# Gadersd/stable-diffusion-burn

Measured on NVIDIA H100. Metric: images_per_sec_512x512_20steps, higher is better.
Workload: dtype fp16 tensor-core operands (3-term split-fp16 on the two high-res UNet levels), fp32 accumulate

## Files before the change

### stable_diffusion_burn_b200/csrc/api.cu

```cuda
#include "../../include/sdb200.h"

#include <dlfcn.h>

#include <cstdlib>
#include <cstring>
#include <mutex>

#include "attention.cuh"
#include "kernels.cuh"
#include "model.cuh"
#include "runtime.cuh"

using namespace sdb;

struct sdb_ctx {
  Ctx c;
};

static thread_local std::string g_err;

#define API_BEGIN(ctxp)                      \
  if (!(ctxp)) {                             \
    g_err = "null context";                  \
    return 1;                                \
// ... 323 lines not shown
                    int L, const float* d_uncond, int Lu, double guidance_scale, int n_steps, const float* d_noise, int H, int W,
                    float* d_latent_out, uint8_t* d_rgb_out, void* stream) {
  API_BEGIN(ctx)
  need_final(c);
  model_img2img_dev(c, d_image, d_mask, strength, d_context, n, L, d_uncond, Lu, guidance_scale, n_steps, d_noise, H, W,
                    d_latent_out, d_rgb_out, (cudaStream_t)stream);
  API_END
}

int sdb_forward_diffuser(sdb_ctx* ctx, const float* latent, int32_t timestep, const float* context, int n, int L,
                         const float* uncond, int Lu, double guidance_scale, int H, int W, float* pred, float* out_uncond,
                         float* out_cond) {
  API_BEGIN(ctx)
  need_final(c);
  SDB_CHECK(latent && context && uncond, "null argument");
  model_forward_diffuser_host(c, latent, timestep, context, n, L, uncond, Lu, guidance_scale, H, W, pred, out_uncond, out_cond);
  API_END
}

int sdb_forward_diffuser_dev(sdb_ctx* ctx, const float* d_latent, int32_t timestep, const float* d_context, int n, int L,
                             const float* d_uncond, int Lu, double guidance_scale, int H, int W, float* d_pred, void* stream) {
  API_BEGIN(ctx)
  need_final(c);
  model_forward_diffuser_dev(c, d_latent, timestep, d_context, n, L, d_uncond, Lu, guidance_scale, H, W, d_pred, nullptr, nullptr,
                             (cudaStream_t)stream);
  API_END
}

int sdb_encode_image(sdb_ctx* ctx, const float* img, int n, int H, int W, float* latent) {
  API_BEGIN(ctx)
  need_final(c);
  SDB_CHECK(img && latent, "null argument");
  model_encode_host(c, img, n, H, W, latent);
  API_END
}

int sdb_encode_image_dev(sdb_ctx* ctx, const float* d_img, int n, int H, int W, float* d_latent, void* stream) {
  API_BEGIN(ctx)
  need_final(c);
  model_encode_dev(c, d_img, n, H, W, d_latent, (cudaStream_t)stream);
  API_END
}

int sdb_clip_forward(sdb_ctx* ctx, const int32_t* tokens, int n, int L, float* out) {
  API_BEGIN(ctx)
  need_final(c);
  SDB_CHECK(tokens && out, "null argument");
  model_clip_forward_host(c, tokens, n, L, out);
  API_END
}

int sdb_clip_forward_dev(sdb_ctx* ctx, const int32_t* d_tokens, int n, int L, float* d_out, void* stream) {
  API_BEGIN(ctx)
  need_final(c);
  model_clip_forward_dev(c, d_tokens, n, L, d_out, (cudaStream_t)stream);
  API_END
}

int sdb_set_option(sdb_ctx* ctx, const char* key, int value) {
  API_BEGIN(ctx)
  const std::string k = key ? key : "";
  if (k == "precision")
    c.opt_precision = value;
  else if (k == "graphs")
    c.opt_graphs = value;
  else if (k == "splitk")
    c.opt_splitk = value;
  else if (k == "raw16")
    c.opt_raw16 = value;
  else if (k == "splitk_min_iters")
    c.opt_splitk_min_iters = value;
  else if (k == "splitk_chunk")
    c.opt_splitk_chunk = value < 1 ? 1 : value;
  else if (k == "attn_split")
    c.opt_attn_split = value;
  else if (k == "attn_regsplit")
    g_attn_regsplit = value;
  else if (k == "emb_hoist")
    c.opt_emb_hoist = value;
  else if (k == "prefetch_w")
    c.opt_prefetch_w = value;
  else if (k == "mlp_passes")
    c.opt_mlp_passes = value;
  else if (k == "gn_epilogue")
    c.opt_gn_epilogue = value;
  else if (k == "skip_merge")
    c.opt_skip_merge = value;
  else if (k == "gn_apply_ctas")
    g_gn_apply_ctas = value < 1 ? 1 : value;
  else if (k == "gn_min_pix")
    g_gn_min_pix = value < 1 ? 1 : value;
  else
    throw Error("unknown option: " + k);
  model_invalidate_graphs(c);
  API_END
}

int sdb_profile_enable(sdb_ctx* ctx, int on) {
  API_BEGIN(ctx)
  profile_collect(c);
  c.profiling = on != 0;
  API_END
}
int sdb_profile_reset(sdb_ctx* ctx) {
  API_BEGIN(ctx)
  profile_collect(c);
  c.launches = 0;
  for (int i = 0; i < KC_COUNT; ++i) c.cls_ms[i] = c.cls_flops[i] = c.cls_bytes[i] = c.cls_issued[i] = 0, c.cls_launches[i] = 0;
  API_END
}
int sdb_profile_class_count(sdb_ctx*) { return KC_COUNT; }
int sdb_profile_get(sdb_ctx* ctx, int cls, const char** name, int64_t* launches, double* ms, double* flops, double* bytes) {
  API_BEGIN(ctx)
  SDB_CHECK(cls >= 0 && cls < KC_COUNT, "class index");
  profile_collect(c);
  if (name) *name = kernel_class_name(cls);
  if (launches) *launches = c.cls_launches[cls];
  if (ms) *ms = c.cls_ms[cls];
  if (flops) *flops = c.cls_flops[cls];
  if (bytes) *bytes = c.cls_bytes[cls];
  API_END
}
int sdb_profile_get_issued(sdb_ctx* ctx, int cls, double* issued_flops) {
  API_BEGIN(ctx)
  SDB_CHECK(cls >= 0 && cls < KC_COUNT && issued_flops, "class index");
  *issued_flops = c.cls_issued[cls];
  API_END
}
int64_t sdb_launch_count(sdb_ctx* ctx) { return ctx ? ctx->c.launches : -1; }

int sdb_test_linear(sdb_ctx* ctx, const float* a, const float* w, const float* bias, int M, int K, int N, int passes,
                    float* out) {
  API_BEGIN(ctx)
  c.work.reset();
  float* d_a = c.work.get<float>((size_t)M * K);
  float* d_w = c.work.get<float>((size_t)K * N);
  float* d_b = bias ? c.work.get<float>(N) : nullptr;
  float* d_c = c.work.get<float>((size_t)M * N);
  SDB_CUDA(cudaMemcpyAsync(d_a, a, sizeof(float) * M * K, cudaMemcpyHostToDevice, c.stream));
  SDB_CUDA(cudaMemcpyAsync(d_w, w, sizeof(float) * K * N, cudaMemcpyHostToDevice, c.stream));
  if (bias) SDB_CUDA(cudaMemcpyAsync(d_b, bias, sizeof(float) * N, cudaMemcpyHostToDevice, c.stream));
  ActOp A;
  A.p.hi = c.work.get<__half>((size_t)M * K);
  A.p.lo = c.work.get<__half>((size_t)M * K);
  A.W = M, A.C = K;
  WeightOp Wp;
  Wp.p.hi = c.work.get<__half>((size_t)N * K);
  Wp.p.lo = c.work.get<__half>((size_t)N * K);
  Wp.N = N, Wp.K = K;
  convert_f16_launch(d_a, (long long)M * K, A.p, c.stream);
  pack_linear_launch(d_w, K, N, Wp.p, 0, c.stream);
  Epilogue ep;
  ep.out_f32 = d_c;
  ep.bias = d_b;
  run_gemm(c, G_LINEAR, A, nullptr, Wp, passes, ep);
  SDB_CUDA(cudaMemcpyAsync(out, d_c, sizeof(float) * M * N, cudaMemcpyDeviceToHost, c.stream));
  SDB_CUDA(cudaStreamSynchronize(c.stream));
  API_END
}

int sdb_test_gemm_ex(sdb_ctx* ctx, const float* a, const float* w, const float* bias, const float* residual, int M, int K, int N,
                     int passes, int flags, const float* xa, const float* xw, int XK, float* out) {
  API_BEGIN(ctx)
  c.work.reset();
  const bool geglu = flags & 1, from_f16 = flags & 4;
  SDB_CHECK(!geglu || (N % 128 == 0 && !residual && !xa), "GEGLU test: N (= 2 * hidden) must be a multiple of 128, no residual / extra K");
// ... 321 lines not shown
```

### stable_diffusion_burn_b200/csrc/gemm_tc.cu

```cuda
#include "gemm_tc.cuh"

#include <cstring>

namespace sdb {

static constexpr int BM = 128;
static constexpr int BK = 64;
static constexpr int A_TILE_BYTES = BM * BK * 2;

template <int BN, int PASSES>
struct StageLayout {
  static constexpr int B_TILE_BYTES = BN * BK * 2;
  static constexpr int A_TILES = PASSES >= 2 ? 2 : 1;
  static constexpr int B_TILES = PASSES >= 3 ? 2 : 1;
  static constexpr int BYTES = A_TILES * A_TILE_BYTES + B_TILES * B_TILE_BYTES;
};
template <int BN>
struct AccLayout {
  static constexpr int PITCH = (BN + 4) * 4;
  static constexpr int BYTES = BM * PITCH;
  static constexpr int GN_BYTES = 32 * 1024;
};
static constexpr int EW = 8;

// ... 559 lines not shown
      if constexpr (kGN) {
        asm volatile("bar.sync 1, %0;" ::"n"(EW * 32) : "memory");
        gn_write_partials(p, gn_cs, BN, threadIdx.x - 128, EW * 32, gnt, col0, p.up2 ? (int)blockIdx.z * p.gn_phase_slots : 0);
      }
    }
    if (dbg && threadIdx.x == 128) dbg[6] = clock64();
  }
  __syncthreads();
  if (dbg && threadIdx.x == 0) dbg[7] = clock64();
}

static constexpr int SMEM_OPTIN_MAX = 227 * 1024;
template <int BN, int PASSES>
constexpr int pick_stages() {
  constexpr int per = StageLayout<BN, PASSES>::BYTES;
  constexpr int n = (SMEM_OPTIN_MAX - 1024) / (per + 2 * 8);
  return n > 8 ? 8 : n;
}

template <int BN, int PASSES, int STAGES, int EPI>
static void launch_epi(const GemmMaps& maps, const GemmParams& p, cudaStream_t stream) {
  constexpr int smem = region_bytes<BN, PASSES, STAGES>() + 2 * STAGES * 8 + 1024;
  static_assert(smem <= SMEM_OPTIN_MAX, "shared memory per block");
  static_assert(4 * BN * 8 <= AccLayout<BN>::GN_BYTES && 2 * (EW * 32) * 4 * 16 <= AccLayout<BN>::GN_BYTES,
                "GroupNorm column sums must fit in the scratch after the accumulator image");
  static DeviceOnce once;
  if (once.first())
    SDB_CUDA(cudaFuncSetAttribute(gemm_tc_kernel<BN, PASSES, STAGES, EPI>, cudaFuncAttributeMaxDynamicSharedMemorySize, smem));
  dim3 grid(p.tiles_n * p.tiles_h * p.tiles_w, (p.N + BN - 1) / BN, p.up2 ? 4 : p.split_k);
  launch_k(gemm_tc_kernel<BN, PASSES, STAGES, EPI>, grid, dim3(128 + 32 * EW), (size_t)smem, stream, maps, p);
}
template <int BN, int PASSES, int STAGES>
static void launch_inst(const GemmMaps& maps, const GemmParams& p, cudaStream_t stream) {
  SDB_CHECK((p.gn_part != nullptr) + (p.ln_out != nullptr) + (p.ln_in != nullptr) <= 1, "one statistics role per launch");
  if constexpr (BN == 128) {
    if (p.geglu) {
      SDB_CHECK(!p.gn_part && !p.ln_out && p.split_k == 1, "GEGLU epilogue: no statistics output, no split-K");
      return p.ln_in ? launch_epi<BN, PASSES, STAGES, EPI_GEGLU_LNC>(maps, p, stream)
                     : launch_epi<BN, PASSES, STAGES, EPI_GEGLU>(maps, p, stream);
    }
  }
  SDB_CHECK(!p.geglu, "the GEGLU epilogue is built for 128-wide tiles");
  if constexpr (BN >= 128) {
    if (p.gn_part) return launch_epi<BN, PASSES, STAGES, EPI_GN>(maps, p, stream);
  }
  if constexpr (BN == 160) {
    if (p.ln_out) return launch_epi<BN, PASSES, STAGES, EPI_LNS>(maps, p, stream);
  }
  if constexpr (BN == 128 || BN == 160) {
    if (p.ln_in) return launch_epi<BN, PASSES, STAGES, EPI_LNC>(maps, p, stream);
  }
  SDB_CHECK(!p.gn_part && !p.ln_out && !p.ln_in, "this statistics epilogue is not built for this tile width");
  launch_epi<BN, PASSES, STAGES, EPI_PLAIN>(maps, p, stream);
}
bool gemm_tc_supports(int BN, int epi) {
  return epi == EPI_PLAIN || (epi == EPI_GN && BN >= 128) || (epi == EPI_LNS && BN == 160) || (epi == EPI_LNC && (BN == 128 || BN == 160));
}

template <int BN, int PASSES>
static void launch_bn(const GemmMaps& maps, const GemmParams& p, cudaStream_t stream) {
  launch_inst<BN, PASSES, pick_stages<BN, PASSES>()>(maps, p, stream);
}

void gemm_tc_launch(const GemmMaps& maps, const GemmParams& p, int BN, int passes, cudaStream_t stream) {
  SDB_CHECK(p.TN * p.TH * p.TW == BM, "M tile must cover 128 rows");
  SDB_CHECK(p.N % 32 == 0, "N must be a multiple of 32");
#define SDB_DISPATCH(bn)                                             \
  case bn:                                                           \
    if (passes == 1) launch_bn<bn, 1>(maps, p, stream);              \
    else if (passes == 2) launch_bn<bn, 2>(maps, p, stream);         \
    else launch_bn<bn, 3>(maps, p, stream);                          \
    break;
  switch (BN) {
    SDB_DISPATCH(64)
    SDB_DISPATCH(128)
    SDB_DISPATCH(160)
    SDB_DISPATCH(256)
    default:
      throw Error("unsupported BN");
  }
#undef SDB_DISPATCH
}

}
```

### stable_diffusion_burn_b200/csrc/gemm_tc.cuh

```cuda
#pragma once
#include "common.cuh"

namespace sdb {

struct GemmMaps {
  CUtensorMap a[4][2];
  CUtensorMap bx[2];
  CUtensorMap b[2];
};

struct GemmParams {
  int nimg, H, W;
  int TN, TH, TW;
  int tiles_n, tiles_h, tiles_w;
  int N;
  int kc;
  int kc0;
  int num_taps;
  int xkc, xkc0;
  int8_t tap_dh[9], tap_dw[9], tap_ph[9];
  int split_k;
  int up2, gn_phase_slots;
  float* out_f32;
  __half* out_f16;
  __half* out_f16_lo;
  const float* bias;
  const float* rowbias;
  const float* residual;
  int ldc;
  int ldc16;
  int geglu;
  long long* dbg;
  int prefetch_w;
  int pdl_late;
  int act;
  float* gn_part;
  int gn_cap, gn_bucket, gn_slot0;
  int gn_rpi, gn_nimg;
  float* ln_out;
  int ln_slots;
  const float* ln_in;
  int ln_in_slots, ln_C;
  float ln_eps;
  const float* ln_u;
  const __half* res_hi;
  const __half* res_lo;
  float* ws;
  unsigned int* tickets;
  int OH, OW, os, oa, ob;
};

struct GemmLaunch {
  int BN, passes, stages;
};

void gemm_tc_launch(const GemmMaps& maps, const GemmParams& p, int BN, int passes, cudaStream_t stream);
bool gemm_tc_supports(int BN, int epi);
int gemm_tc_smem_bytes(int BN, int passes, int stages);

}
```

### stable_diffusion_burn_b200/csrc/runtime.cu

```cuda
#include "runtime.cuh"

#include <algorithm>

#include <cudaTypedefs.h>

#include <cmath>
#include <cstdlib>
#include <cstring>

namespace sdb {

int g_pdl_late = 1;
bool g_pdl_enabled = true;
int g_num_sms = 132;

void Arena::init(size_t bytes) {
  SDB_CUDA(cudaMalloc(&base, bytes));
  cap = bytes;
  off = 0;
}
void Arena::destroy() {
  if (base) cudaFree(base);
  base = nullptr;
  cap = off = 0;
// ... 242 lines not shown
      p.num_taps = 9;
      for (int t = 0; t < 9; ++t) p.tap_dh[t] = t / 3 - 1, p.tap_dw[t] = t % 3 - 1, p.tap_ph[t] = 0;
      break;
    case G_CONV3_S2:
      SDB_CHECK(a0.P == 4, "stride-2 conv needs a 4-phase operand");
      p.num_taps = 9;
      for (int t = 0; t < 9; ++t) {
        const int kh = t / 3, kw = t % 3;
        p.tap_dh[t] = kh == 0 ? -1 : 0;
        p.tap_dw[t] = kw == 0 ? -1 : 0;
        p.tap_ph[t] = (kh != 1 ? 2 : 0) + (kw != 1 ? 1 : 0);
      }
      break;
    case G_CONV3_S2_PAD01:
      SDB_CHECK(a0.P == 4, "stride-2 conv needs a 4-phase operand");
      p.num_taps = 9;
      for (int t = 0; t < 9; ++t) {
        const int kh = t / 3, kw = t % 3;
        p.tap_dh[t] = kh == 2 ? 1 : 0;
        p.tap_dw[t] = kw == 2 ? 1 : 0;
        p.tap_ph[t] = (kh == 1 ? 2 : 0) + (kw == 1 ? 1 : 0);
      }
      break;
    case G_CONV3_UP2:
      p.num_taps = 4;
      phases_out = 4;
      break;
    default:
      throw Error("bad gemm kind");
  }
  SDB_CHECK(w.K == p.num_taps * Ctot, "weight K does not match the operand");
  if (xk) {
    const int xC = xk->x0.C + (xk->has_x1 ? xk->x1.C : 0);
    SDB_CHECK(kind == G_CONV3 || kind == G_LINEAR, "extra-K operands need an unshifted output grid");
    SDB_CHECK(xk->x0.n == a0.n && xk->x0.H == a0.H && xk->x0.W == a0.W && xk->x0.P == 1 && xk->x0.C % 64 == 0, "extra-K geometry");
    SDB_CHECK(!xk->has_x1 || (xk->x1.n == a0.n && xk->x1.H == a0.H && xk->x1.W == a0.W && xk->x1.C % 64 == 0), "extra-K geometry");
    SDB_CHECK(xk->w.N == w.N && xk->w.K == xC, "extra-K weights");
    SDB_CHECK(passes < 2 || (xk->x0.p.lo && (!xk->has_x1 || xk->x1.p.lo)), "multi-pass GEMM needs the lo half of the extra operands");
    SDB_CHECK(passes < 3 || xk->w.p.lo, "3-pass GEMM needs the lo half of the extra weights");
    p.xkc0 = xk->x0.C / 64, p.xkc = xC / 64;
  }

  p.TW = std::min(pow2_floor(a0.W), 128);
  p.TH = std::min(128 / p.TW, pow2_ceil(a0.H));
  p.TN = 128 / (p.TW * p.TH);
  p.tiles_w = (a0.W + p.TW - 1) / p.TW;
  p.tiles_h = (a0.H + p.TH - 1) / p.TH;
  p.tiles_n = (a0.n + p.TN - 1) / p.TN;
  const int m_tiles = p.tiles_w * p.tiles_h * p.tiles_n;

  int BN;
  if (ep.geglu)
    BN = 128;
  else if (w.N % 160 == 0)
    BN = 160;
  else if (w.N % 256 == 0 && (long long)m_tiles * (w.N / 256) >= 2 * g_num_sms)
    BN = 256;
  else if (w.N % 128 == 0)
    BN = 128;
  else
    BN = 64;
  if (ep.ln_out) {
    SDB_CHECK(w.N % 160 == 0 && !ep.geglu, "LayerNorm statistics need an output width that tiles by 160");
    BN = 160;
  }
  if (ep.ln_in) SDB_CHECK(BN == 128 || BN == 160, "LayerNorm-consuming GEMM: tile width");
  const int n_tiles = (w.N + BN - 1) / BN;


  const int iters = p.num_taps * p.kc + p.xkc;
  int split = 1;
  if (c.opt_splitk && kind != G_CONV3_UP2 && !ep.geglu && !ep.ln_out && !ep.ln_in) {
    const int ctas = m_tiles * n_tiles;
    if (ctas <= g_num_sms / 2 && iters >= c.opt_splitk_min_iters) {
      split = std::min(std::min(g_num_sms / ctas, iters / c.opt_splitk_chunk), 16);
      if (split < 1) split = 1;
    }
  }
  if (split > 1) {
    const int per = (iters + split - 1) / split;
    split = (iters + per - 1) / per;
  }
  p.split_k = split;
  static const bool gemm_dbg = getenv("SDB_GEMM_DBG") != nullptr || getenv("SDB_LABEL_LOG") != nullptr;
  if (c.debug_sync || c.profiling || gemm_dbg) {
    char buf[256];
    snprintf(buf, sizeof(buf), "gemm kind=%d n=%d H=%d W=%d P=%d C0=%d C1=%d N=%d K=%d xk=%d BN=%d split=%d passes=%d geglu=%d epi=%s%s tile=%dx%dx%d",
             kind, a0.n, a0.H, a0.W, a0.P, a0.C, a1in ? a1.C : 0, w.N, w.K, p.xkc * 64, BN, split, passes, ep.geglu,
             ep.gn ? "gn" : (ep.ln_out ? "lns" : (ep.ln_in ? "lnc" : "-")), ep.residual16.hi ? "+r16" : (ep.residual ? "+r32" : ""), p.TN, p.TH, p.TW);
    c.dbg_label = buf;
  }

  GnPart* gn = ep.gn;
  if (gn) {
    int slots = m_tiles / p.tiles_n * split * phases_out;
    bool geom = p.TN <= 4;
    if (kind == G_LINEAR && gn_rpi > 0) {
      const long long rows = (long long)a0.W;
      geom = rows % gn_rpi == 0 && (gn_rpi % 128 == 0 || (128 % gn_rpi == 0 && gn_rpi >= 32));
      gn_nimg = (int)(rows / gn_rpi);
      slots = (gn_rpi >= 128 ? gn_rpi / 128 : 1) * split;
    } else {
      if (kind == G_LINEAR) geom = false;
      gn_rpi = 0;
    }
    const bool ok = gn->buf && gn->bucket > 0 && !ep.geglu && geom && BN >= 128 && BN % gn->bucket == 0 && w.N % gn->bucket == 0 &&
                    slots <= gn->cap && c.opt_gn_epilogue;
    gn->slots = ok ? slots : 0;
    if (!ok) gn = nullptr;
  }
  if (c.trace_on)
    c.gemm_trace.push_back({kind_in, w.N, BN, split, p.TN, p.TH, p.TW, p.xkc * 64, gn ? gn->slots : 0, a1in ? a1.C : 0});
  p.gn_part = gn ? gn->buf : nullptr;
  p.gn_cap = gn ? gn->cap : 0, p.gn_bucket = gn ? gn->bucket : 1;
  p.gn_rpi = gn ? gn_rpi : 0, p.gn_nimg = gn_nimg;
  p.ln_out = ep.ln_out, p.ln_slots = ln_slots(w.N);
  p.ln_in = ep.ln_in, p.ln_in_slots = ep.ln_in_slots, p.ln_C = ep.ln_C, p.ln_eps = ep.ln_eps;
  p.ln_u = passes >= 3 ? ep.ln_u_full : ep.ln_u_hi;
  SDB_CHECK(!ep.ln_in || (p.ln_u && ep.ln_in_slots > 0 && ep.ln_C == w.K && kind == G_LINEAR), "LayerNorm-consuming GEMM: arguments");
  SDB_CHECK(!ep.ln_in || (!ep.residual && !ep.rowbias && !ep.residual16.hi), "LayerNorm-consuming GEMM: no residual / row bias");
  SDB_CHECK(!ep.ln_out || kind == G_LINEAR, "LayerNorm statistics: rows must be tokens");
  p.res_hi = ep.residual16.hi, p.res_lo = ep.residual16.lo;
  SDB_CHECK(!ep.residual16.hi || (ep.residual16.lo && !ep.residual && !ep.rowbias), "fp16-pair residual: needs both halves, excludes the fp32 residual / row bias");
  p.out_f32 = ep.out_f32;
  p.out_f16 = ep.out_f16.hi;
  p.out_f16_lo = ep.out_f16.lo;
  p.bias = ep.bias;
  p.rowbias = ep.rowbias;
  p.residual = ep.residual;
  p.geglu = ep.geglu;
  p.act = ep.act;
  p.pdl_late = g_pdl_late;
  p.prefetch_w = (g_pdl_enabled && c.opt_prefetch_w && m_tiles <= 4) ? 1 : 0;
  const int nout = ep.geglu ? w.N / 2 : w.N;
  p.ldc = ep.ldc ? ep.ldc : nout;
  p.ldc16 = ep.ldc16 ? ep.ldc16 : nout;
  SDB_CHECK(!(ep.rowbias && ep.residual), "epilogue takes a time-embedding row or a residual, not both");
  p.os = (kind == G_CONV3_UP2) ? 2 : 1;
  p.OH = a0.H * p.os, p.OW = a0.W * p.os;
  SDB_CHECK((double)a0.n * p.OH * p.OW * (double)std::max(p.ldc, p.ldc16) < 2147483648.0,
            "GEMM output exceeds 2^31 elements (the epilogue uses 32-bit element offsets)");

  GemmMaps maps;
  memset(&maps, 0, sizeof(maps));
  maps.a[0][0] = make_act_map(a0.p.hi, a0.C, a0.W, a0.H, a0.P, a0.n, p.TW, p.TH, p.TN);
  maps.a[0][1] = maps.a[0][0];
  if (passes >= 2) maps.a[0][1] = make_act_map(a0.p.lo, a0.C, a0.W, a0.H, a0.P, a0.n, p.TW, p.TH, p.TN);
  maps.a[1][0] = maps.a[0][0];
  maps.a[1][1] = maps.a[0][1];
  if (a1in) {
    SDB_CHECK(a1.n == a0.n && a1.H == a0.H && a1.W == a0.W && a1.P == a0.P, "concat operand geometry");
    maps.a[1][0] = make_act_map(a1.p.hi, a1.C, a1.W, a1.H, a1.P, a1.n, p.TW, p.TH, p.TN);
    maps.a[1][1] = maps.a[1][0];
    if (passes >= 2) maps.a[1][1] = make_act_map(a1.p.lo, a1.C, a1.W, a1.H, a1.P, a1.n, p.TW, p.TH, p.TN);
  }

  for (int sidx = 2; sidx < 4; ++sidx) maps.a[sidx][0] = maps.a[sidx][1] = maps.a[0][0];
  if (xk) {
    auto xmaps = [&](const ActOp& x, int sidx) {
      maps.a[sidx][0] = make_act_map(x.p.hi, x.C, x.W, x.H, x.P, x.n, p.TW, p.TH, p.TN);
      maps.a[sidx][1] = passes >= 2 ? make_act_map(x.p.lo, x.C, x.W, x.H, x.P, x.n, p.TW, p.TH, p.TN) : maps.a[sidx][0];
    };
    xmaps(xk->x0, 2);
    if (xk->has_x1) xmaps(xk->x1, 3);
  }

  const double Mtot = (double)a0.n * a0.H * a0.W;
  const double flops = 2.0 * Mtot * (double)w.N * ((double)w.K + 64.0 * p.xkc);
  const double a_bytes = Mtot * (Ctot + 64.0 * p.xkc) * 2.0 * (passes >= 2 ? 2 : 1);
  const double w_bytes = (double)w.N * (w.K + 64.0 * p.xkc) * 2.0 * (passes >= 3 ? 2 : 1);
  const double o_bytes = Mtot * nout * ((ep.out_f32 ? 4.0 : 0.0) + (ep.out_f16.hi ? 2.0 : 0.0) + (ep.out_f16.lo ? 2.0 : 0.0)) +
                         (ep.residual ? Mtot * nout * 4.0 : 0.0);
  const double bytes = a_bytes + w_bytes + o_bytes;

  {
    const __half* whi = w.p.hi;
    const __half* wlo = w.p.lo;
    const int wrows = (w.rows ? w.rows : w.N) * phases_out;
    const int bbox = BN;
    maps.b[0] = make_w_map(whi, w.K, wrows, bbox, w.ld);
    maps.b[1] = maps.b[0];
    if (passes >= 3) maps.b[1] = make_w_map(wlo, w.K, wrows, bbox, w.ld);
    maps.bx[0] = maps.bx[1] = maps.b[0];
    if (xk) {
      const int xrows = xk->w.rows ? xk->w.rows : xk->w.N;
      maps.bx[0] = make_w_map(xk->w.p.hi, xk->w.K, xrows, bbox, xk->w.ld);
      maps.bx[1] = passes >= 3 ? make_w_map(xk->w.p.lo, xk->w.K, xrows, bbox, xk->w.ld) : maps.bx[0];
    }
    p.gn_slot0 = 0;
    p.up2 = 0, p.gn_phase_slots = (m_tiles / p.tiles_n) * split;
    if (kind == G_CONV3_UP2) {
      p.up2 = 1, p.oa = 0, p.ob = 0;
      for (int t = 0; t < 4; ++t) p.tap_dh[t] = (t >> 1) - 1, p.tap_dw[t] = (t & 1) - 1, p.tap_ph[t] = 0;
    }
    if (split > 1) {
      const size_t need = (size_t)split * (size_t)Mtot * w.N * sizeof(float);
      p.ws = reinterpret_cast<float*>(c.work.alloc(need));
      SDB_CHECK((long long)m_tiles * n_tiles * 2 <= 65536, "split-K ticket buffer");
      SDB_CHECK((long long)m_tiles * n_tiles * split <= g_num_sms, "split-K CTAs must be co-resident");
      p.tickets = c.splitk_tickets;
    }
    {
      static const bool dbg_on = getenv("SDB_GEMM_DBG") != nullptr;
      static long long* dbg_buf = nullptr;
      if (dbg_on) {
        if (!dbg_buf) SDB_CUDA(cudaMallocManaged(&dbg_buf, 16 * sizeof(long long)));
        SDB_CUDA(cudaStreamSynchronize(c.stream));
        memset(dbg_buf, 0, 16 * sizeof(long long));
        p.dbg = dbg_buf;
      }
      const std::string label = c.dbg_label;
      {
        KernelScope ks(c, KC_GEMM, flops * phases_out, bytes * phases_out, flops * passes * phases_out);
        gemm_tc_launch(maps, p, BN, passes, c.stream);
      }
      if (dbg_on) {
        SDB_CUDA(cudaStreamSynchronize(c.stream));
        fprintf(stderr, "gemm_dbg %s | cycles since entry: prologue %lld tma0 %lld landed %lld lastmma %lld accum %lld epi %lld exit %lld | chunk0: ld %lld stage %lld finish %lld (bias %lld loads0 %lld batch0 %lld)\n",
                label.c_str(), dbg_buf[1] - dbg_buf[0], dbg_buf[2] - dbg_buf[0], dbg_buf[3] - dbg_buf[0],
                dbg_buf[4] - dbg_buf[0], dbg_buf[5] - dbg_buf[0], dbg_buf[6] - dbg_buf[0], dbg_buf[7] - dbg_buf[0], dbg_buf[9] - dbg_buf[8], dbg_buf[10] - dbg_buf[9],
                dbg_buf[11] - dbg_buf[10], dbg_buf[12] - dbg_buf[10], dbg_buf[13] - dbg_buf[12], dbg_buf[14] - dbg_buf[13]);
      }
    }
  }
}

}
```

### stable_diffusion_burn_b200/csrc/runtime.cuh

```cuda
#pragma once
#include <string>
#include <unordered_map>
#include <unordered_set>
#include <vector>

#include "common.cuh"
#include "attention.cuh"
#include "gemm_tc.cuh"
#include "kernels.cuh"

namespace sdb {

struct Arena {
  char* base = nullptr;
  size_t cap = 0, off = 0, high = 0;
  void init(size_t bytes);
  void destroy();
  void* alloc(size_t bytes);
  template <class T>
  T* get(size_t count) {
    return reinterpret_cast<T*>(alloc(count * sizeof(T)));
  }
  void reset() { off = 0; }
};
// ... 19 lines not shown
  KC_PREP,
  KC_LAYERNORM,
  KC_SMALLCONV,
  KC_ELEMENTWISE,
  KC_COUNT
};

struct ProfEvent {
  int cls;
  cudaEvent_t a, b;
  double flops, bytes;
  std::string label;
};

struct ActOp {
  Half2Ptr p;
  int n = 1, P = 1, H = 1, W = 1, C = 0;
};
struct WeightOp {
  Half2Ptr p;
  int N = 0, K = 0;
  long long ld = 0;
  int rows = 0;
};
enum GemmKind : int { G_LINEAR = 0, G_CONV1 = 1, G_CONV3 = 2, G_CONV3_S2 = 3, G_CONV3_UP2 = 4, G_CONV3_S2_PAD01 = 5 };

struct GnPart {
  float* buf = nullptr;
  int cap = 0, bucket = 0, slots = 0;
};

struct Epilogue {
  float* ln_out = nullptr;
  const float* ln_in = nullptr;
  int ln_in_slots = 0, ln_C = 0;
  float ln_eps = 1e-5f;
  const float* ln_u_hi = nullptr;
  const float* ln_u_full = nullptr;
  Half2Ptr residual16;
  GnPart* gn = nullptr;
  int gn_rpi = 0;
  float* out_f32 = nullptr;
  Half2Ptr out_f16;
  const float* bias = nullptr;
  const float* rowbias = nullptr;
  const float* residual = nullptr;
  int geglu = 0;
  int act = 0;
  int ldc = 0;
  int ldc16 = 0;
};

struct MetaCheck {
  std::string relpath;
  std::vector<float> values;
  bool must_be_absent = false;
};

constexpr int kIoImg2ImgZ0 = 8;
constexpr int kIoImg2ImgW = 9;

struct Ctx {
  int device = 0;
  cudaStream_t stream = nullptr;
  bool own_stream = true;
  std::string err;
  Arena master, packed, work;
  std::vector<TensorInfo> tensors;
  std::unordered_map<std::string, int> index;
  bool finalized = false;
  std::vector<MetaCheck> meta;
  std::unordered_set<std::string> group_norms;
  std::unordered_map<std::string, float> norm_eps;
  int opt_precision = 0;
  int opt_graphs = 1;
  int opt_splitk = 1;
  int opt_splitk_min_iters = 32, opt_splitk_chunk = 8;
  int opt_skip_merge = 1;
  int opt_raw16 = 1;
  int opt_mlp_passes = 0;
  int opt_attn_split = 1;
  int opt_emb_hoist = 1;
  int opt_prefetch_w = 0;
  int opt_gn_epilogue = 1;
  bool profiling = false;
  std::vector<ProfEvent> prof;
  int64_t launches = 0;
  double cls_ms[KC_COUNT] = {0}, cls_flops[KC_COUNT] = {0}, cls_bytes[KC_COUNT] = {0};
  double cls_issued[KC_COUNT] = {0};
  int64_t cls_launches[KC_COUNT] = {0};
  struct IoBuf {
    void* p = nullptr;
    size_t cap = 0;
  } iobuf[10];
  void* io(int slot, size_t bytes);
  void io_destroy();
  void* model = nullptr;
  unsigned int* splitk_tickets = nullptr;
  bool debug_sync = false;
  std::string dbg_label;
  struct GemmRecord {
    int kind, N, BN, split, TN, TH, TW, xk_channels, gn_slots, a1_channels;
  };
  bool trace_on = false;
  std::vector<GemmRecord> gemm_trace;
  std::vector<int> gn_trace;

  float* master_ptr(const std::string& name);
  const TensorInfo& info(const std::string& name);
  bool has(const std::string& name) const { return index.count(name) != 0; }
};

struct KernelScope {
  Ctx& c;
  int cls;
  bool on;
  ProfEvent ev;
  KernelScope(Ctx& c, int cls, double flops = 0, double bytes = 0, double issued = 0);
  ~KernelScope();
};
void profile_collect(Ctx& c);

struct ExtraK {
  ActOp x0, x1;
  bool has_x1 = false;
  WeightOp w;
};

void run_gemm(Ctx& c, int kind, const ActOp& a0, const ActOp* a1, const WeightOp& w, int passes, const Epilogue& ep,
              const ExtraK* xk = nullptr);

struct AttnOp {
  const __half* q = nullptr;
  int ldq = 0, q_col0 = 0, q_rows = 0;
  const __half* k = nullptr;
  int ldk = 0, k_col0 = 0, k_rows = 0;
  const __half* q_lo = nullptr;
  const __half* k_lo = nullptr;
  const __half* vT = nullptr;
  int ldv = 0;
  int v_mn = 0, v_col0 = 0;
  int nb = 1, heads = 8, d = 0, dpad = 0, Nq = 0, Nk = 0;
  const int* kvlen = nullptr;
  int causal = 0;
  Half2Ptr out;
  int ldo = 0;
};
void run_attention(Ctx& c, const AttnOp& a);
inline int ln_slots(int N) { return ((N + 159) / 160) * 2; }

const char* kernel_class_name(int cls);

}
```

Before: 3.939.

## Add persistent 64-row GEMM kernel with overlapped epilogue for LayerNorm/GEGLU linears

Adds a persistent warp-specialized GEMM kernel for 3-pass linear layers using 64-row tiles. One producer warp streams TMA loads across several tiles, and two consumer warpgroups alternate tiles so that one group's epilogue overlaps the other's MMA. It is enabled by default for linears with LayerNorm-stats, LayerNorm-consume or GEGLU epilogues. The aim is to hide epilogue latency and reduce wave quantization, at the cost of smaller M tiles and extra named-barrier synchronization.

Result: faster. 4.006, median of 6 (+1.7%).

```diff
diff --git a/stable_diffusion_burn_b200/csrc/api.cu b/stable_diffusion_burn_b200/csrc/api.cu
--- a/stable_diffusion_burn_b200/csrc/api.cu
+++ b/stable_diffusion_burn_b200/csrc/api.cu
@@ -429,6 +429,8 @@
     c.opt_prefetch_w = value;
   else if (k == "mlp_passes")
     c.opt_mlp_passes = value;
+  else if (k == "gemm_persistent")
+    c.opt_gemm_persistent = value;
   else if (k == "gn_epilogue")
     c.opt_gn_epilogue = value;
   else if (k == "skip_merge")
diff --git a/stable_diffusion_burn_b200/csrc/gemm_tc.cu b/stable_diffusion_burn_b200/csrc/gemm_tc.cu
--- a/stable_diffusion_burn_b200/csrc/gemm_tc.cu
+++ b/stable_diffusion_burn_b200/csrc/gemm_tc.cu
@@ -665,4 +665,400 @@
 #undef SDB_DISPATCH
 }
 
-}
+template <int BN, int PASSES>
+struct PpLayout {
+  static constexpr int A_BYTES = 64 * BK * 2;
+  static constexpr int A_TILES = PASSES >= 2 ? 2 : 1;
+  static constexpr int B_TILES = PASSES >= 3 ? 2 : 1;
+  static constexpr int STAGE = A_TILES * A_BYTES + B_TILES * BN * BK * 2;
+  static constexpr int IMG = 64 * AccLayout<BN>::PITCH;
+};
+template <int BN, int PASSES, int STAGES, int NIMG>
+constexpr int pp_smem_bytes() {
+  return STAGES * PpLayout<BN, PASSES>::STAGE + NIMG * PpLayout<BN, PASSES>::IMG + 2 * STAGES * 8 + 1024;
+}
+
+template <int BN, int PASSES, int STAGES, int NIMG, int EPI>
+__global__ void __launch_bounds__(128 + 32 * EW, 1)
+gemm_pp_kernel(const __grid_constant__ GemmMaps maps, const GemmParams p) {
+  constexpr bool kLNS = EPI == EPI_LNS, kLNC = EPI == EPI_LNC || EPI == EPI_GEGLU_LNC;
+  constexpr bool kGEGLU = EPI == EPI_GEGLU || EPI == EPI_GEGLU_LNC;
+  static_assert(EPI != EPI_GN, "GroupNorm partials are written per 128-row tile: one-tile kernel only");
+  using L = PpLayout<BN, PASSES>;
+  constexpr int CSTEP = 64;
+  extern __shared__ __align__(1024) uint8_t smem_raw[];
+  uint8_t* smem = smem_raw + ((1024u - (smem_u32(smem_raw) & 1023u)) & 1023u);
+  uint64_t* full_bar = reinterpret_cast<uint64_t*>(smem + STAGES * L::STAGE + NIMG * L::IMG);
+  uint64_t* empty_bar = full_bar + STAGES;
+
+  const int warp = threadIdx.x >> 5;
+  const int lane = threadIdx.x & 31;
+  long long* const dbg = (p.dbg && blockIdx.x == 0) ? p.dbg : nullptr;
+  if (dbg && threadIdx.x == 0) dbg[0] = clock64();
+  if (!p.pdl_late) pdl_trigger();
+
+  const int n_tiles = (p.N + BN - 1) / BN;
+  const int tiles = p.tiles_w * n_tiles;
+  const int my_tiles = (int)blockIdx.x < tiles ? (tiles - 1 - (int)blockIdx.x) / (int)gridDim.x + 1 : 0;
+  const int iters = p.kc;
+
+  if (threadIdx.x == 0) {
+    for (int s = 0; s < STAGES; ++s) {
+      mbar_init(&full_bar[s], 1);
+      mbar_init(&empty_bar[s], 4);
+    }
+    fence_mbar_init();
+  }
+  if (warp == 0 && lane == 0) {
+    tma_prefetch_desc(&maps.a[0][0]);
+    tma_prefetch_desc(&maps.b[0]);
+    if (p.kc0 < p.kc) tma_prefetch_desc(&maps.a[1][0]);
+  }
+  __syncthreads();
+  if (dbg && threadIdx.x == 0) dbg[1] = clock64();
+  if (warp == 0) {
+    if (elect_one() && my_tiles > 0) {
+      auto load_b = [&](int it, int n0, int s) {
+        uint8_t* sb = smem + s * L::STAGE + L::A_TILES * L::A_BYTES;
+        tma_load_2d(sb, &maps.b[0], &full_bar[s], it * BK, n0);
+        if (PASSES >= 3) tma_load_2d(sb + BN * BK * 2, &maps.b[1], &full_bar[s], it * BK, n0);
+      };
+      auto load_a = [&](int it, int m0, int s) {
+        const int src = it >= p.kc0 ? 1 : 0;
+        const int c0 = (it - (src ? p.kc0 : 0)) * BK;
+        uint8_t* st = smem + s * L::STAGE;
+        tma_load_5d(st, &maps.a[src][0], &full_bar[s], c0, m0, 0, 0, 0);
+        if (PASSES >= 2) tma_load_5d(st + L::A_BYTES, &maps.a[src][1], &full_bar[s], c0, m0, 0, 0, 0);
+      };
+      int t = blockIdx.x;
+      const int npre = min(STAGES, iters);
+      for (int i = 0; i < npre; ++i) {
+        mbar_expect_tx(&full_bar[i], L::STAGE);
+        load_b(i, (t % n_tiles) * BN, i);
+      }
+      pdl_wait();
+      for (int i = 0; i < npre; ++i) load_a(i, (t / n_tiles) * 64, i);
+      if (dbg) dbg[2] = clock64();
+      int s = npre == STAGES ? 0 : npre;
+      uint32_t ph = npre == STAGES ? 1 : 0;
+      int it = npre;
+      for (int i = 0; i < my_tiles; ++i, t += gridDim.x, it = 0) {
+        const int m0 = (t / n_tiles) * 64, n0 = (t % n_tiles) * BN;
+        for (; it < iters; ++it) {
+          mbar_wait(&empty_bar[s], ph ^ 1);
+          mbar_expect_tx(&full_bar[s], L::STAGE);
+          load_a(it, m0, s);
+          load_b(it, n0, s);
+          if (++s == STAGES) {
+            s = 0;
+            ph ^= 1;
+          }
+        }
+      }
+    }
+  } else if (warp >= 4) {
+    pdl_wait();
+    const int wg = (warp - 4) >> 2;
+    const int q = warp & 1;
+    const int half = (warp >> 1) & 1;
+    const uint32_t img_base = smem_u32(smem + STAGES * L::STAGE + (NIMG == 2 ? wg : 0) * L::IMG);
+    const int bar_wg = 4 + wg;
+    constexpr uint32_t TROW = AccLayout<BN>::PITCH;
+    const int sub = lane >> 3;
+    const int cq = (lane & 7) * 4;
+    constexpr int NCHUNK = (BN + CSTEP - 1) / CSTEP;
+#pragma unroll 1
+    for (int i = wg; i < my_tiles; i += 2) {
+      const int t = blockIdx.x + i * gridDim.x;
+      const int nt = t % n_tiles, m0 = (t / n_tiles) * 64, col0 = nt * BN;
+      float acc[BN / 2];
+      if (i > 0) {
+        if (wg == 0) asm volatile("bar.sync 6, 256;" ::: "memory");
+        else asm volatile("bar.sync 7, 256;" ::: "memory");
+      }
+      {
+#pragma unroll
+        for (int k = 0; k < BN / 2; ++k) acc[k] = 0.f;
+        const int g0 = i * iters;
+        int s = g0 % STAGES, prev = -1;
+        uint32_t ph = (g0 / STAGES) & 1;
+        for (int it = 0; it < iters; ++it) {
+          mbar_wait(&full_bar[s], ph);
+          if (dbg && threadIdx.x == 128 && i == 0 && it == 0) dbg[3] = clock64();
+          const uint32_t a_hi = smem_u32(smem + s * L::STAGE);
+          const uint32_t a_lo = a_hi + L::A_BYTES;
+          const uint32_t b_hi = a_hi + L::A_TILES * L::A_BYTES;
+          const uint32_t b_lo = b_hi + BN * BK * 2;
+          wgmma_fence();
+#pragma unroll
+          for (int k = 0; k < BK / 16; ++k) {
+            const uint32_t koff = k * 32;
+            const uint64_t da = make_sdesc_sw128(a_hi + koff);
+            const uint64_t db = make_sdesc_sw128(b_hi + koff);
+            Wgmma<BN>::template ss<0>(acc, da, db, 1);
+            if (PASSES >= 2) Wgmma<BN>::template ss<0>(acc, make_sdesc_sw128(a_lo + koff), db, 1);
+            if (PASSES >= 3) Wgmma<BN>::template ss<0>(acc, da, make_sdesc_sw128(b_lo + koff), 1);
+          }
+          wgmma_commit();
+          wgmma_wait<1>();
+          if (prev >= 0 && lane == 0) mbar_arrive(&empty_bar[prev]);
+          prev = s;
+          if (++s == STAGES) {
+            s = 0;
+            ph ^= 1;
+          }
+        }
+        if (i + 1 < my_tiles) {
+          if (wg == 0) asm volatile("bar.arrive 7, 256;" ::: "memory");
+          else asm volatile("bar.arrive 6, 256;" ::: "memory");
+        }
+        wgmma_wait<0>();
+        reg_fence(acc);
+        if (lane == 0) mbar_arrive(&empty_bar[prev]);
+      }
+      if (dbg && threadIdx.x == 128 && i == 0) dbg[4] = clock64();
+      if (NIMG == 1 && i > 0) {
+        if (wg == 0) asm volatile("bar.sync 2, 256;" ::: "memory");
+        else asm volatile("bar.sync 3, 256;" ::: "memory");
+      }
+      if (NIMG == 2 && i >= 2) asm volatile("bar.sync %0, 128;" ::"r"(bar_wg) : "memory");
+      {
+        float* img = reinterpret_cast<float*>(smem + STAGES * L::STAGE + (NIMG == 2 ? wg : 0) * L::IMG);
+        const int r0 = (warp & 3) * 16 + (lane >> 2);
+#pragma unroll
+        for (int j = 0; j < BN / 2; j += 2) {
+          const int row = r0 + 8 * ((j >> 1) & 1), col = 8 * (j >> 2) + 2 * (lane & 3);
+          *reinterpret_cast<float2*>(img + row * (TROW / 4) + col) = make_float2(acc[j], acc[j + 1]);
+        }
+      }
+      asm volatile("bar.sync %0, 128;" ::"r"(bar_wg) : "memory");
+
+      const int r = q * 32 + lane;
+      const int m = m0 + r < p.W ? m0 + r : -1;
+      int mr8[8], ao[8];
+      float4 bvs[NCHUNK], ad[8];
+      const float* ad_ptr = p.residual ? p.residual : p.rowbias;
+      const bool res_pair = p.res_hi != nullptr;
+      float ln_mu = 0.f, ln_rs = 0.f;
+      float mu8[8], rs8[8];
+      float4 us[NCHUNK];
+      if constexpr (kLNC) {
+        if (m >= 0) {
+          const float2* sp = reinterpret_cast<const float2*>(p.ln_in) + (size_t)m * p.ln_in_slots;
+          float sm = 0.f, sq = 0.f;
+          for (int k = 0; k < p.ln_in_slots; ++k) {
+            const float2 v = sp[k];
+            sm += v.x, sq += v.y;
+          }
+          const float inv = 1.0f / (float)p.ln_C;
+          ln_mu = sm * inv;
+          ln_rs = rsqrtf(fmaxf(sq * inv - ln_mu * ln_mu, 0.f) + p.ln_eps);
+        }
+      }
+      {
+        const bool use_res = p.residual != nullptr;
+#pragma unroll
+        for (int k = 0; k < 8; ++k) {
+          const int rr = k * 4 + sub;
+          const int mr = __shfl_sync(0xffffffffu, m, rr);
+          mr8[k] = mr;
+          ao[k] = res_pair ? mr * p.ldc16 : (use_res ? mr * p.ldc : 0);
+          ad[k] = make_float4(0.f, 0.f, 0.f, 0.f);
+          if constexpr (kLNC) mu8[k] = __shfl_sync(0xffffffffu, ln_mu, rr), rs8[k] = __shfl_sync(0xffffffffu, ln_rs, rr);
+        }
+        if constexpr (kLNC) {
+#pragma unroll
+          for (int j = 0; j < NCHUNK; ++j) {
+            const int col = col0 + half * 32 + j * CSTEP + cq;
+            us[j] = make_float4(0.f, 0.f, 0.f, 0.f);
+            if (half * 32 + j * CSTEP < BN && col < p.N) us[j] = *reinterpret_cast<const float4*>(p.ln_u + col);
+          }
+        }
+#pragma unroll
+        for (int j = 0; j < NCHUNK; ++j) {
+          const int col = col0 + half * 32 + j * CSTEP + cq;
+          bvs[j] = make_float4(0.f, 0.f, 0.f, 0.f);
+          if (!kGEGLU && p.bias && half * 32 + j * CSTEP < BN && col < p.N) bvs[j] = *reinterpret_cast<const float4*>(p.bias + col);
+        }
+      }
+      auto issue_addends = [&](int col) {
+        if constexpr (kLNC) return;
+        if (col >= p.N) return;
+        if (res_pair) {
+#pragma unroll
+          for (int k = 0; k < 8; ++k)
+            if (mr8[k] >= 0) {
+              const uint2 h = *reinterpret_cast<const uint2*>(p.res_hi + (unsigned)(ao[k] + col));
+              const uint2 l = *reinterpret_cast<const uint2*>(p.res_lo + (unsigned)(ao[k] + col));
+              const float2 h0 = __half22float2(*reinterpret_cast<const __half2*>(&h.x)), h1 = __half22float2(*reinterpret_cast<const __half2*>(&h.y));
+              const float2 l0 = __half22float2(*reinterpret_cast<const __half2*>(&l.x)), l1 = __half22float2(*reinterpret_cast<const __half2*>(&l.y));
+              ad[k] = make_float4(h0.x + l0.x, h0.y + l0.y, h1.x + l1.x, h1.y + l1.y);
+            }
+          return;
+        }
+        if (ad_ptr == nullptr) return;
+#pragma unroll
+        for (int k = 0; k < 8; ++k)
+          if (mr8[k] >= 0) ad[k] = *reinterpret_cast<const float4*>(ad_ptr + (unsigned)(ao[k] + col));
+      };
+      if (!kGEGLU) issue_addends(col0 + half * 32 + cq);
+      if (p.pdl_late && i == my_tiles - 1) pdl_trigger();
+      if (dbg && threadIdx.x == 128 && i == 0) dbg[5] = clock64();
+      const uint32_t arow = img_base + q * 32 * TROW;
+
+      if constexpr (kGEGLU) {
+        constexpr int HB = BN / 2;
+        const int ocol0 = nt * HB;
+        auto unstage = [&](uint32_t a, int rr) {
+          float4 f;
+          asm volatile("ld.shared.v4.f32 {%0, %1, %2, %3}, [%4];"
+                       : "=f"(f.x), "=f"(f.y), "=f"(f.z), "=f"(f.w)
+                       : "r"(a + rr * TROW + cq * 4)
+                       : "memory");
+          return f;
+        };
+#pragma unroll 1
+        for (int c = half * 32; c < HB; c += CSTEP) {
+          const float4 bx = *reinterpret_cast<const float4*>(p.bias + col0 + c + cq);
+          const float4 bg = *reinterpret_cast<const float4*>(p.bias + col0 + HB + c + cq);
+          float4 ux = make_float4(0.f, 0.f, 0.f, 0.f), ug = ux;
+          if constexpr (kLNC) {
+            ux = *reinterpret_cast<const float4*>(p.ln_u + col0 + c + cq);
+            ug = *reinterpret_cast<const float4*>(p.ln_u + col0 + HB + c + cq);
+          }
+#pragma unroll 1
+          for (int k = 0; k < 8; ++k) {
+            const int rr = k * 4 + sub;
+            const int mr = __shfl_sync(0xffffffffu, m, rr);
+            float rmu = 0.f, rrs = 1.f;
+            if constexpr (kLNC) rmu = __shfl_sync(0xffffffffu, ln_mu, rr), rrs = __shfl_sync(0xffffffffu, ln_rs, rr);
+            if (mr >= 0) {
+              float4 tx = unstage(arow + c * 4, rr), tg = unstage(arow + (HB + c) * 4, rr);
+              if constexpr (kLNC) {
+                tx.x = rrs * (tx.x - rmu * ux.x), tx.y = rrs * (tx.y - rmu * ux.y), tx.z = rrs * (tx.z - rmu * ux.z), tx.w = rrs * (tx.w - rmu * ux.w);
+                tg.x = rrs * (tg.x - rmu * ug.x), tg.y = rrs * (tg.y - rmu * ug.y), tg.z = rrs * (tg.z - rmu * ug.z), tg.w = rrs * (tg.w - rmu * ug.w);
+              }
+              float4 y;
+              y.x = (tx.x + bx.x) * gelu_erf_fast(tg.x + bg.x);
+              y.y = (tx.y + bx.y) * gelu_erf_fast(tg.y + bg.y);
+              y.z = (tx.z + bx.z) * gelu_erf_fast(tg.z + bg.z);
+              y.w = (tx.w + bx.w) * gelu_erf_fast(tg.w + bg.w);
+              epilogue_store(y, 0u, (unsigned)(mr * p.ldc16 + ocol0 + c + cq), nullptr, p.out_f16, p.out_f16_lo, 0);
+            }
+          }
+        }
+      } else {
+        float lrs[8], lrq[8];
+#pragma unroll
+        for (int k = 0; k < 8; ++k) lrs[k] = 0.f, lrq[k] = 0.f;
+        (void)lrs, (void)lrq;
+#pragma unroll
+        for (int j = 0; j < NCHUNK; ++j) {
+          const int c = half * 32 + j * CSTEP;
+          if (c < BN) {
+            const int col = col0 + c + cq;
+            if (col < p.N) {
+              const uint32_t tl = arow + c * 4 + sub * TROW + cq * 4;
+#pragma unroll
+              for (int b4 = 0; b4 < 2; ++b4) {
+                float4 tv[4];
+#pragma unroll
+                for (int k = 0; k < 4; ++k)
+                  asm volatile("ld.shared.v4.f32 {%0, %1, %2, %3}, [%4];"
+                               : "=f"(tv[k].x), "=f"(tv[k].y), "=f"(tv[k].z), "=f"(tv[k].w)
+                               : "r"(tl + (b4 * 4 + k) * 4 * TROW)
+                               : "memory");
+#pragma unroll
+                for (int k4 = 0; k4 < 4; ++k4) {
+                  const int k = b4 * 4 + k4;
+                  if (mr8[k] < 0) continue;
+                  float4 f = tv[k4];
+                  if constexpr (kLNC) {
+                    f.x = rs8[k] * (f.x - mu8[k] * us[j].x), f.y = rs8[k] * (f.y - mu8[k] * us[j].y);
+                    f.z = rs8[k] * (f.z - mu8[k] * us[j].z), f.w = rs8[k] * (f.w - mu8[k] * us[j].w);
+                  }
+                  if constexpr (kLNC)
+                    f.x += bvs[j].x, f.y += bvs[j].y, f.z += bvs[j].z, f.w += bvs[j].w;
+                  else
+                    f.x += bvs[j].x + ad[k].x, f.y += bvs[j].y + ad[k].y, f.z += bvs[j].z + ad[k].z, f.w += bvs[j].w + ad[k].w;
+                  if constexpr (kLNS) {
+                    lrs[k] += (f.x + f.y) + (f.z + f.w);
+                    lrq[k] = fmaf(f.x, f.x, fmaf(f.y, f.y, fmaf(f.z, f.z, fmaf(f.w, f.w, lrq[k]))));
+                  }
+                  epilogue_store(f, (unsigned)(mr8[k] * p.ldc + col), (unsigned)(mr8[k] * p.ldc16 + col), p.out_f32, p.out_f16,
+                                 p.out_f16_lo, p.act);
+                }
+              }
+            }
+            if (j + 1 < NCHUNK && c + CSTEP < BN) issue_addends(col0 + c + CSTEP + cq);
+          }
+        }
+        if constexpr (kLNS) {
+#pragma unroll
+          for (int k = 0; k < 8; ++k) {
+#pragma unroll
+            for (int o = 1; o <= 4; o <<= 1) {
+              lrs[k] += __shfl_xor_sync(0xffffffffu, lrs[k], o);
+              lrq[k] += __shfl_xor_sync(0xffffffffu, lrq[k], o);
+            }
+          }
+          if ((lane & 7) == 0) {
+            const int slot = nt * 2 + half;
+#pragma unroll
+            for (int k = 0; k < 8; ++k)
+              if (mr8[k] >= 0) reinterpret_cast<float2*>(p.ln_out)[(size_t)mr8[k] * p.ln_slots + slot] = make_float2(lrs[k], lrq[k]);
+          }
+        }
+      }
+      if (dbg && threadIdx.x == 128 && i == 0) dbg[6] = clock64();
+      if (NIMG == 1 && i + 1 < my_tiles) {
+        if (wg == 0) asm volatile("bar.arrive 3, 256;" ::: "memory");
+        else asm volatile("bar.arrive 2, 256;" ::: "memory");
+      }
+    }
+  }
+  __syncthreads();
+  if (dbg && threadIdx.x == 0) dbg[7] = clock64();
+}
+
+template <int BN, int PASSES, int STAGES, int NIMG, int EPI>
+static void launch_pp_epi(const GemmMaps& maps, const GemmParams& p, int ctas, cudaStream_t stream) {
+  constexpr int smem = pp_smem_bytes<BN, PASSES, STAGES, NIMG>();
+  static_assert(smem <= SMEM_OPTIN_MAX, "shared memory per block");
+  static DeviceOnce once;
+  if (once.first())
+    SDB_CUDA(cudaFuncSetAttribute(gemm_pp_kernel<BN, PASSES, STAGES, NIMG, EPI>, cudaFuncAttributeMaxDynamicSharedMemorySize, smem));
+  launch_k(gemm_pp_kernel<BN, PASSES, STAGES, NIMG, EPI>, dim3(ctas), dim3(128 + 32 * EW), (size_t)smem, stream, maps, p);
+}
+template <int BN, int STAGES, int NIMG>
+static void launch_pp_bn(const GemmMaps& maps, const GemmParams& p, int ctas, cudaStream_t stream) {
+  if constexpr (BN == 128) {
+    if (p.geglu)
+      return p.ln_in ? launch_pp_epi<BN, 3, STAGES, NIMG, EPI_GEGLU_LNC>(maps, p, ctas, stream)
+                     : launch_pp_epi<BN, 3, STAGES, NIMG, EPI_GEGLU>(maps, p, ctas, stream);
+  }
+  SDB_CHECK(!p.geglu, "the GEGLU epilogue is built for 128-wide tiles");
+  if constexpr (BN == 160) {
+    if (p.ln_out) return launch_pp_epi<BN, 3, STAGES, NIMG, EPI_LNS>(maps, p, ctas, stream);
+  }
+  if (p.ln_in) return launch_pp_epi<BN, 3, STAGES, NIMG, EPI_LNC>(maps, p, ctas, stream);
+  SDB_CHECK(!p.ln_out, "LayerNorm statistics are built for 160-wide tiles");
+  launch_pp_epi<BN, 3, STAGES, NIMG, EPI_PLAIN>(maps, p, ctas, stream);
+}
+
+bool gemm_pp_supports(int BN, int passes) { return passes == 3 && (BN == 128 || BN == 160); }
+
+void gemm_pp_launch(const GemmMaps& maps, const GemmParams& p, int BN, int passes, int num_sms, cudaStream_t stream) {
+  SDB_CHECK(gemm_pp_supports(BN, passes), "persistent GEMM: 3 passes, BN 128 or 160");
+  SDB_CHECK(p.TN == 1 && p.TH == 1 && p.TW == 64 && p.nimg == 1 && p.H == 1 && p.num_taps == 1 && p.xkc == 0 && p.split_k == 1 &&
+                !p.gn_part && !p.up2 && !p.rowbias,
+            "persistent GEMM: 64-row Linear tiles, no extra K, split-K, GroupNorm statistics or row bias");
+  const long long tiles = (long long)p.tiles_w * ((p.N + BN - 1) / BN);
+  const int ctas = (int)std::min<long long>(tiles, num_sms);
+  if (BN == 128)
+    launch_pp_bn<128, 3, 2>(maps, p, ctas, stream);
+  else
+    launch_pp_bn<160, 3, 1>(maps, p, ctas, stream);
+}
+
+}
diff --git a/stable_diffusion_burn_b200/csrc/gemm_tc.cuh b/stable_diffusion_burn_b200/csrc/gemm_tc.cuh
--- a/stable_diffusion_burn_b200/csrc/gemm_tc.cuh
+++ b/stable_diffusion_burn_b200/csrc/gemm_tc.cuh
@@ -55,6 +55,8 @@
 };
 
 void gemm_tc_launch(const GemmMaps& maps, const GemmParams& p, int BN, int passes, cudaStream_t stream);
+void gemm_pp_launch(const GemmMaps& maps, const GemmParams& p, int BN, int passes, int num_sms, cudaStream_t stream);
+bool gemm_pp_supports(int BN, int passes);
 bool gemm_tc_supports(int BN, int epi);
 int gemm_tc_smem_bytes(int BN, int passes, int stages);
 
diff --git a/stable_diffusion_burn_b200/csrc/runtime.cu b/stable_diffusion_burn_b200/csrc/runtime.cu
--- a/stable_diffusion_burn_b200/csrc/runtime.cu
+++ b/stable_diffusion_burn_b200/csrc/runtime.cu
@@ -348,12 +348,20 @@
     split = (iters + per - 1) / per;
   }
   p.split_k = split;
+  bool pp = false;
+  if (c.opt_gemm_persistent && kind == G_LINEAR && split == 1 && !xk && !ep.gn && !ep.rowbias && a0.n == 1 && a0.H == 1 &&
+      a0.P == 1 && gemm_pp_supports(BN, passes) && (c.opt_gemm_persistent == 2 || ep.ln_out || ep.ln_in || ep.geglu)) {
+    const long long tiles64 = (long long)((a0.W + 63) / 64) * n_tiles;
+    pp = BN == 128 || tiles64 <= g_num_sms;
+  }
+  if (pp) p.TN = 1, p.TH = 1, p.TW = 64, p.tiles_n = 1, p.tiles_h = 1, p.tiles_w = (a0.W + 63) / 64;
   static const bool gemm_dbg = getenv("SDB_GEMM_DBG") != nullptr || getenv("SDB_LABEL_LOG") != nullptr;
   if (c.debug_sync || c.profiling || gemm_dbg) {
     char buf[256];
-    snprintf(buf, sizeof(buf), "gemm kind=%d n=%d H=%d W=%d P=%d C0=%d C1=%d N=%d K=%d xk=%d BN=%d split=%d passes=%d geglu=%d epi=%s%s tile=%dx%dx%d",
+    snprintf(buf, sizeof(buf), "gemm kind=%d n=%d H=%d W=%d P=%d C0=%d C1=%d N=%d K=%d xk=%d BN=%d split=%d passes=%d geglu=%d epi=%s%s tile=%dx%dx%d%s",
              kind, a0.n, a0.H, a0.W, a0.P, a0.C, a1in ? a1.C : 0, w.N, w.K, p.xkc * 64, BN, split, passes, ep.geglu,
-             ep.gn ? "gn" : (ep.ln_out ? "lns" : (ep.ln_in ? "lnc" : "-")), ep.residual16.hi ? "+r16" : (ep.residual ? "+r32" : ""), p.TN, p.TH, p.TW);
+             ep.gn ? "gn" : (ep.ln_out ? "lns" : (ep.ln_in ? "lnc" : "-")), ep.residual16.hi ? "+r16" : (ep.residual ? "+r32" : ""), p.TN, p.TH, p.TW,
+             pp ? " pp" : "");
     c.dbg_label = buf;
   }
 
@@ -478,7 +486,10 @@
       const std::string label = c.dbg_label;
       {
         KernelScope ks(c, KC_GEMM, flops * phases_out, bytes * phases_out, flops * passes * phases_out);
-        gemm_tc_launch(maps, p, BN, passes, c.stream);
+        if (pp)
+          gemm_pp_launch(maps, p, BN, passes, g_num_sms, c.stream);
+        else
+          gemm_tc_launch(maps, p, BN, passes, c.stream);
       }
       if (dbg_on) {
         SDB_CUDA(cudaStreamSynchronize(c.stream));
diff --git a/stable_diffusion_burn_b200/csrc/runtime.cuh b/stable_diffusion_burn_b200/csrc/runtime.cuh
--- a/stable_diffusion_burn_b200/csrc/runtime.cuh
+++ b/stable_diffusion_burn_b200/csrc/runtime.cuh
@@ -125,6 +125,7 @@
   int opt_attn_split = 1;
   int opt_emb_hoist = 1;
   int opt_prefetch_w = 0;
+  int opt_gemm_persistent = 1;
   int opt_gn_epilogue = 1;
   bool profiling = false;
   std::vector<ProfEvent> prof;
```
